# sczhou/Upscale-A-Video

Hardware: NVIDIA H100
Metric: upscaled frames/sec (30 DDIM steps, 180x320->4x) (higher is better)
Workload: dtype f16

## Files before the change

### upscale_a_video_b200/csrc/igemm.cu

```cuda
#include <stdarg.h>
#include <stdlib.h>
#include <stdio.h>
#include <string.h>

#include <atomic>
#include <mutex>

#include "uav_common.cuh"

namespace uav {

static thread_local char g_err[1024] = "";
void set_last_error(const char* fmt, ...) {
  va_list ap;
  va_start(ap, fmt);
  vsnprintf(g_err, sizeof(g_err), fmt, ap);
  va_end(ap);
}
std::atomic<uint64_t> g_launches{0};

int current_device() {
  int dev = 0;
  cudaGetDevice(&dev);
  return dev;
}

int num_sms() {
  static int n[64] = {0};
  const int dev = current_device() & 63;
  if (n[dev] == 0) {
    int v = 0;
    cudaDeviceGetAttribute(&v, cudaDevAttrMultiProcessorCount, dev);
    n[dev] = v > 0 ? v : 132;
  }
  return n[dev];
}

PFN_encodeTiled get_encode_tiled() {
  static PFN_encodeTiled fn = nullptr;
  static std::once_flag once;
  std::call_once(once, [] {
    void* p = nullptr;
    cudaDriverEntryPointQueryResult qres;
    if (cudaGetDriverEntryPoint("cuTensorMapEncodeTiled", &p, cudaEnableDefault, &qres) ==
            cudaSuccess &&
        qres == cudaDriverEntryPointSuccess)
      fn = reinterpret_cast<PFN_encodeTiled>(p);
  });
  return fn;
}

constexpr int BLOCK_M = 128;
constexpr int BLOCK_K = 64;
constexpr int MAX_TAPS = 49;
constexpr int NUM_THREADS = 384;
constexpr int NUM_EPI_THREADS = 256;
constexpr int A_STAGE_BYTES = BLOCK_M * BLOCK_K * 2;
constexpr int SLAB_BYTES = BLOCK_M * 128;
constexpr int SMEM_LIMIT = 232448;

struct alignas(64) IgemmParams {
  CUtensorMap map_a;
  CUtensorMap map_b;
  CUtensorMap map_out;
  CUtensorMap map_res;
  int32_t tap_off[MAX_TAPS][5];
  int32_t num_taps;
  int32_t kblocks_per_tap;
  int32_t k_per_tap;
  uint32_t box[5];
  uint32_t tiles[5];
  uint32_t out_dims[5];
  uint32_t n_tiles, num_tiles;
  int32_t N;
  int32_t n_out;
  int32_t tma_store;
  int32_t res_tma;
  const float* bias;
  const __half* rowvec;
  int64_t rows_per_vec, ld_rowvec;
  const __half* residual;
  int64_t ld_res;
  int32_t act, out_dtype;
  int64_t ld_out;
  void* out;
  float out_scale;
  float* gn_partial;
  int64_t gn_blocks;
};

template <int BLOCK_N, bool GEGLU>
struct IgemmCfg {
  static constexpr int OUT_TILE_N = GEGLU ? BLOCK_N / 2 : BLOCK_N;
  static constexpr int B_STAGE_BYTES = BLOCK_N * BLOCK_K * 2;
  static constexpr int STAGE_BYTES = A_STAGE_BYTES + B_STAGE_BYTES;
  static constexpr int STAGING_BYTES = (OUT_TILE_N >= 64) ? (OUT_TILE_N / 64) * SLAB_BYTES : 0;
  static constexpr int AUX_BYTES = 1024;
  static constexpr int STAGES_RAW = (SMEM_LIMIT - 1024 - STAGING_BYTES - AUX_BYTES) / STAGE_BYTES;
  static constexpr int STAGES = STAGES_RAW > 8 ? 8 : STAGES_RAW;
  static constexpr int SMEM_BYTES = STAGES * STAGE_BYTES + STAGING_BYTES + AUX_BYTES + 1024 ;
  static constexpr int ACC = BLOCK_N / 2;
};

__device__ __forceinline__ void epi_bar_sync() {
  asm volatile("bar.sync 1, %0;" ::"n"(NUM_EPI_THREADS) : "memory");
}
__device__ __forceinline__ float apply_act(float x, int act) {
  switch (act) {
    case UAV_ACT_SILU: return silu_f(x);
    case UAV_ACT_RELU: return fmaxf(x, 0.f);
    case UAV_ACT_SIGMOID: return rcp_ftz(1.0f + ex2_ftz(-1.4426950408889634f * x));
    case UAV_ACT_TANH: return 1.0f - 2.0f * rcp_ftz(1.0f + ex2_ftz(2.8853900817779268f * x));
    case UAV_ACT_GELU: return gelu_erf_f(x);
    case UAV_ACT_QUICK_GELU: return x * rcp_ftz(1.0f + ex2_ftz(-2.4554669595930156f * x));
    default: return x;
  }
}
__device__ __forceinline__ float warp_sum(float v) {
#pragma unroll
  for (int o = 16; o >= 1; o >>= 1) v += __shfl_xor_sync(0xffffffffu, v, o);
  return v;
}

template <int BLOCK_N, bool GEGLU, bool TMA_EPI, bool AUX>
__global__ void __launch_bounds__(NUM_THREADS, 1)
    igemm_kernel(const __grid_constant__ IgemmParams p) {
  using Cfg = IgemmCfg<BLOCK_N, GEGLU>;
  static_assert(!TMA_EPI || Cfg::OUT_TILE_N >= 64, "TMA-store epilogue needs >= 64-column output tiles");
  constexpr int OUT_TILE_N = Cfg::OUT_TILE_N;
  constexpr int STAGES = Cfg::STAGES;
  extern __shared__ uint8_t smem_raw[];
  const uint32_t raw_addr = smem_u32(smem_raw);
  uint8_t* smem = smem_raw + (((raw_addr + 1023u) & ~1023u) - raw_addr);
  uint8_t* staging = smem + STAGES * Cfg::STAGE_BYTES;
  uint64_t* bars = reinterpret_cast<uint64_t*>(staging + Cfg::STAGING_BYTES);
  uint64_t* full_bar = bars;
  uint64_t* empty_bar = bars + STAGES;
  uint64_t* res_bar = bars + 2 * STAGES;

  const int warp_idx = threadIdx.x >> 5;
  const int lane = threadIdx.x & 31;

  if (threadIdx.x == 0) {
    tma_prefetch_desc(&p.map_a);
    tma_prefetch_desc(&p.map_b);
    if (TMA_EPI) tma_prefetch_desc(&p.map_out);
    if (TMA_EPI && p.res_tma) tma_prefetch_desc(&p.map_res);
    for (int s = 0; s < STAGES; ++s) {
      mbar_init(&full_bar[s], 1);
      mbar_init(&empty_bar[s], NUM_EPI_THREADS / 32);
    }
    mbar_init(res_bar, 1);
    fence_barrier_init();
  }
  __syncthreads();
  const int num_kb = p.num_taps * p.kblocks_per_tap;

  if (warp_idx < 4) {
    if (threadIdx.x == 0) {
      int stage = 0;
      uint32_t phase = 0;
      for (uint32_t w = blockIdx.x; w < p.num_tiles; w += gridDim.x) {
        const uint32_t n_tile = w % p.n_tiles;
        uint32_t idx = w / p.n_tiles;
        const int c1 = (idx % p.tiles[1]) * p.box[1];
        idx /= p.tiles[1];
        const int c2 = (idx % p.tiles[2]) * p.box[2];
        idx /= p.tiles[2];
        const int c3 = (idx % p.tiles[3]) * p.box[3];
        idx /= p.tiles[3];
        const int c4 = idx * p.box[4];
        for (int tap = 0; tap < p.num_taps; ++tap) {
          const int o0 = p.tap_off[tap][0], o1 = p.tap_off[tap][1], o2 = p.tap_off[tap][2],
                    o3 = p.tap_off[tap][3], o4 = p.tap_off[tap][4];
          for (int kc = 0; kc < p.kblocks_per_tap; ++kc) {
            mbar_wait(&empty_bar[stage], phase ^ 1);
            uint8_t* sa = smem + stage * Cfg::STAGE_BYTES;
            uint8_t* sb = sa + A_STAGE_BYTES;
            mbar_expect_tx(&full_bar[stage], Cfg::STAGE_BYTES);
            tma_load_5d(&p.map_a, &full_bar[stage], sa, kc * BLOCK_K + o0, c1 + o1, c2 + o2, c3 + o3, c4 + o4);
            const int kcoord = tap * p.k_per_tap + kc * BLOCK_K;
            if (GEGLU) {
              tma_load_2d(&p.map_b, &full_bar[stage], sb, kcoord, n_tile * (BLOCK_N / 2));
              tma_load_2d(&p.map_b, &full_bar[stage], sb + Cfg::B_STAGE_BYTES / 2, kcoord,
                          p.N / 2 + n_tile * (BLOCK_N / 2));
            } else {
              tma_load_2d(&p.map_b, &full_bar[stage], sb, kcoord, n_tile * BLOCK_N);
            }
            if (++stage == STAGES) {
              stage = 0;
              phase ^= 1;
            }
          }
        }
      }
    }
    return;
  }

  const int et = threadIdx.x - 128;
  const int wg = et >> 7;
  const int cw = et >> 5;
  const int lq = lane >> 2, lr = lane & 3;
  uint32_t lrow[2], l1[2], l2[2], l3[2], l4[2];
#pragma unroll
  for (int h = 0; h < 2; ++h) {
    uint32_t r = 16 * cw + lq + 8 * h;
    lrow[h] = r;
    l1[h] = r % p.box[1];
    r /= p.box[1];
    l2[h] = r % p.box[2];
    r /= p.box[2];
    l3[h] = r % p.box[3];
    r /= p.box[3];
    l4[h] = r;
  }
  int stage = 0;
  uint32_t phase = 0, res_phase = 0;
  float acc[Cfg::ACC];
#pragma unroll
  for (int i = 0; i < Cfg::ACC; ++i) acc[i] = 0.f;

  for (uint32_t w = blockIdx.x; w < p.num_tiles; w += gridDim.x) {
    const uint32_t n_tile = w % p.n_tiles;
    const uint32_t m_tile = w / p.n_tiles;
    uint32_t idx = m_tile;
    const uint32_t t1 = (idx % p.tiles[1]) * p.box[1];
    idx /= p.tiles[1];
    const uint32_t t2 = (idx % p.tiles[2]) * p.box[2];
    idx /= p.tiles[2];
    const uint32_t t3 = (idx % p.tiles[3]) * p.box[3];
    idx /= p.tiles[3];
    const uint32_t t4 = idx * p.box[4];
    const int n_base = n_tile * OUT_TILE_N;

    if constexpr (TMA_EPI) {
      if (et == 0) {
        asm volatile("cp.async.bulk.wait_group.read 0;" ::: "memory");
        if (AUX && p.res_tma) {
          uint32_t bytes = 0;
#pragma unroll
          for (int sl = 0; sl < OUT_TILE_N / 64; ++sl)
            if (n_base + sl * 64 < p.n_out) bytes += SLAB_BYTES;
          mbar_expect_tx(res_bar, bytes);
#pragma unroll
          for (int sl = 0; sl < OUT_TILE_N / 64; ++sl)
            if (n_base + sl * 64 < p.n_out)
              tma_load_5d(&p.map_res, res_bar, staging + sl * SLAB_BYTES, n_base + sl * 64, (int)t1, (int)t2, (int)t3,
                          (int)t4);
        }
      }
    }

    int prev = 0;
    for (int kb = 0; kb < num_kb; ++kb) {
      mbar_wait(&full_bar[stage], phase);
      const uint32_t sa = smem_u32(smem + stage * Cfg::STAGE_BYTES) + wg * (64 * 128);
      const uint32_t sb = smem_u32(smem + stage * Cfg::STAGE_BYTES + A_STAGE_BYTES);
      const uint64_t adesc = gmma_desc_sw128(sa), bdesc = gmma_desc_sw128(sb);
      wgmma_fence();
#pragma unroll
      for (int k = 0; k < BLOCK_K / 16; ++k) wgmma_ss(acc, adesc + 2 * k, bdesc + 2 * k, (kb | k) != 0);
      wgmma_commit();
      if (kb > 0) {
        wgmma_wait<1>();
        if (lane == 0) mbar_arrive(&empty_bar[prev]);
      }
      prev = stage;
      if (++stage == STAGES) {
        stage = 0;
        phase ^= 1;
      }
    }
    wgmma_wait<0>();
    wgmma_fence_operands(acc);
    if (lane == 0) mbar_arrive(&empty_bar[prev]);

    bool row_ok[2];
    int64_t out_row[2];
    const __half* rv[2];
    const __half* res[2];
#pragma unroll
    for (int h = 0; h < 2; ++h) {
      const uint32_t o1 = t1 + l1[h], o2 = t2 + l2[h], o3 = t3 + l3[h], o4 = t4 + l4[h];
      row_ok[h] = o1 < p.out_dims[1] && o2 < p.out_dims[2] && o3 < p.out_dims[3] && o4 < p.out_dims[4];
      out_row[h] = ((static_cast<int64_t>(o4) * p.out_dims[3] + o3) * p.out_dims[2] + o2) * p.out_dims[1] + o1;
      rv[h] = (AUX && p.rowvec != nullptr && row_ok[h]) ? p.rowvec + (out_row[h] / p.rows_per_vec) * p.ld_rowvec
                                                         : nullptr;
      res[h] = (AUX && !TMA_EPI && p.residual != nullptr && row_ok[h]) ? p.residual + out_row[h] * p.ld_res : nullptr;
    }
    if constexpr (TMA_EPI) {
      epi_bar_sync();
      if constexpr (AUX) {
        if (p.res_tma) {
          mbar_wait(res_bar, res_phase);
          res_phase ^= 1;
        }
      }
    }
#pragma unroll
    for (int jb = 0; jb < OUT_TILE_N / 8; ++jb) {
      const int col = jb * 8 + 2 * lr;
      const int n = n_base + col;
      const bool ok0 = n < p.n_out, ok1 = n + 1 < p.n_out;
      float b0 = 0.f, b1 = 0.f, g0 = 0.f, g1 = 0.f;
      if (p.bias != nullptr) {
        if (ok0) b0 = __ldg(p.bias + n);
        if (ok1) b1 = __ldg(p.bias + n + 1);
        if (GEGLU) {
          if (ok0) g0 = __ldg(p.bias + p.N / 2 + n);
          if (ok1) g1 = __ldg(p.bias + p.N / 2 + n + 1);
        }
      }
      float gs = 0.f, gq = 0.f;
#pragma unroll
      for (int h = 0; h < 2; ++h) {
        const float a0 = acc[4 * jb + 2 * h], a1 = acc[4 * jb + 2 * h + 1];
        float x0, x1;
        if constexpr (GEGLU) {
          constexpr int GJ = OUT_TILE_N / 8;
          const float q0 = acc[4 * (jb + GJ) + 2 * h], q1 = acc[4 * (jb + GJ) + 2 * h + 1];
          x0 = (a0 + b0) * gelu_erf_f(q0 + g0);
          x1 = (a1 + b1) * gelu_erf_f(q1 + g1);
        } else {
          x0 = a0 + b0;
          x1 = a1 + b1;
        }
        const uint32_t row = lrow[h];
        uint8_t* sp = staging + (col >> 6) * SLAB_BYTES + row * 128 + ((((col & 63) >> 3) ^ (row & 7)) << 4) + (col & 7) * 2;
        if constexpr (AUX) {
          if (rv[h] != nullptr) {
            if (ok0) x0 += __half2float(rv[h][n]);
            if (ok1) x1 += __half2float(rv[h][n + 1]);
          }
          if (p.act != UAV_ACT_NONE) {
            x0 = apply_act(x0, p.act);
            x1 = apply_act(x1, p.act);
          }
          if (TMA_EPI && p.res_tma) {
            const float2 r = __half22float2(*reinterpret_cast<const __half2*>(sp));
            x0 = fmaf(x0, p.out_scale, r.x);
            x1 = fmaf(x1, p.out_scale, r.y);
          } else if (res[h] != nullptr) {
            x0 = fmaf(x0, p.out_scale, ok0 ? __half2float(res[h][n]) : 0.f);
            x1 = fmaf(x1, p.out_scale, ok1 ? __half2float(res[h][n + 1]) : 0.f);
          } else if (p.out_scale != 1.0f) {
            x0 *= p.out_scale;
            x1 *= p.out_scale;
          }
          if (row_ok[h] && ok0) {
            gs += x0 + x1;
            gq = fmaf(x0, x0, fmaf(x1, x1, gq));
          }
        }
        if constexpr (TMA_EPI) {
          *reinterpret_cast<uint32_t*>(sp) = pack_half2_sat(x0, x1);
        } else if (row_ok[h]) {
          if (p.out_dtype == UAV_F16) {
            __half* op = reinterpret_cast<__half*>(p.out) + out_row[h] * p.ld_out + n;
            if (ok0) op[0] = __float2half_rn(fminf(fmaxf(x0, -65504.f), 65504.f));
            if (ok1) op[1] = __float2half_rn(fminf(fmaxf(x1, -65504.f), 65504.f));
          } else {
            float* op = reinterpret_cast<float*>(p.out) + out_row[h] * p.ld_out + n;
            if (ok0) op[0] = x0;
            if (ok1) op[1] = x1;
          }
        }
      }
      if constexpr (AUX && TMA_EPI) {
        if (p.gn_partial != nullptr) {
          gs = warp_sum(gs);
          gq = warp_sum(gq);
          const int oct = (n_base >> 3) + jb;
          const int64_t blk = static_cast<int64_t>(m_tile) * 8 + cw;
          if (lane == 0 && blk < p.gn_blocks && oct * 8 < p.n_out) {
            p.gn_partial[(static_cast<int64_t>(oct) * p.gn_blocks + blk) * 2] = gs;
            p.gn_partial[(static_cast<int64_t>(oct) * p.gn_blocks + blk) * 2 + 1] = gq;
          }
        }
      }
    }
    if constexpr (TMA_EPI) {
      fence_proxy_async();
      epi_bar_sync();
      if (et == 0) {
#pragma unroll
        for (int sl = 0; sl < OUT_TILE_N / 64; ++sl) {
          if (n_base + sl * 64 < p.n_out) {
            asm volatile(
                "cp.async.bulk.tensor.5d.global.shared::cta.bulk_group"
                " [%0, {%2, %3, %4, %5, %6}], [%1];" ::"l"(reinterpret_cast<uint64_t>(&p.map_out)),
                "r"(smem_u32(staging + sl * SLAB_BYTES)), "r"(n_base + sl * 64), "r"(t1), "r"(t2), "r"(t3), "r"(t4)
                : "memory");
          }
        }
        asm volatile("cp.async.bulk.commit_group;" ::: "memory");
      }
    }
  }
  if (TMA_EPI && et == 0) asm volatile("cp.async.bulk.wait_group.read 0;" ::: "memory");
}

struct IgemmDesc {
  const void* a;
  int rank_a;
  uint64_t a_dims[5];
  uint64_t a_strides[5];
  uint32_t box[5];
  uint32_t tiles[5];
  uint32_t out_dims[5];
  int num_taps;
  int32_t tap_off[MAX_TAPS][5];
  int k_per_tap;
  const void* w;
  int64_t N;
  void* out;
  const uav_epilogue_t* epi;
  uint64_t out_strides[5];
};

template <int BLOCK_N, bool GEGLU, bool TMA_EPI, bool AUX>
static uav_status_t launch_instance2(IgemmParams& p, cudaStream_t stream) {
  using Cfg = IgemmCfg<BLOCK_N, GEGLU>;
  static uint64_t configured = 0;
  const uint64_t dev_bit = 1ull << (current_device() & 63);
  auto kern = igemm_kernel<BLOCK_N, GEGLU, TMA_EPI, AUX>;
  if (!(configured & dev_bit)) {
    UAV_CHECK_CUDA(cudaFuncSetAttribute(kern, cudaFuncAttributeMaxDynamicSharedMemorySize, Cfg::SMEM_BYTES));
    configured |= dev_bit;
  }
  const uint32_t sms = (uint32_t)num_sms();
  kern<<<p.num_tiles < sms ? p.num_tiles : sms, NUM_THREADS, Cfg::SMEM_BYTES, stream>>>(p);
  UAV_CHECK_CUDA(cudaGetLastError());
  g_launches.fetch_add(1, std::memory_order_relaxed);
  return UAV_OK;
}

template <int BLOCK_N, bool GEGLU>
static uav_status_t launch_instance(IgemmParams& p, cudaStream_t stream) {
  const bool aux = p.rowvec != nullptr || p.residual != nullptr || (p.act != UAV_ACT_NONE && p.act != UAV_ACT_GEGLU) ||
                   p.out_scale != 1.0f || p.gn_partial != nullptr;
  if constexpr (IgemmCfg<BLOCK_N, GEGLU>::OUT_TILE_N >= 64) {
    if (p.tma_store) {
      return aux ? launch_instance2<BLOCK_N, GEGLU, true, true>(p, stream)
                 : launch_instance2<BLOCK_N, GEGLU, true, false>(p, stream);
    }
  }
  return launch_instance2<BLOCK_N, GEGLU, false, true>(p, stream);
}

static uav_status_t launch_igemm(const IgemmDesc& d, cudaStream_t stream) {
  const uav_epilogue_t* e = d.epi;
  UAV_REQUIRE(e != nullptr, "igemm: epilogue descriptor is NULL");
  UAV_REQUIRE(d.a && d.w && d.out, "igemm: null pointer");
  UAV_REQUIRE(d.k_per_tap > 0 && d.k_per_tap % 8 == 0,
              "igemm: input channels (%d) must be a positive multiple of 8", d.k_per_tap);
  UAV_REQUIRE((reinterpret_cast<uintptr_t>(d.a) & 15) == 0 &&
                  (reinterpret_cast<uintptr_t>(d.w) & 15) == 0,
              "igemm: operands must be 16-byte aligned");
  const bool geglu = e->act == UAV_ACT_GEGLU;
  UAV_REQUIRE(!geglu || (d.N % 128 == 0), "igemm: GEGLU needs N %% 128 == 0 (N=%lld)",
              (long long)d.N);
  PFN_encodeTiled encode = get_encode_tiled();
  UAV_REQUIRE(encode != nullptr, "igemm: cuTensorMapEncodeTiled entry point unavailable");

  IgemmParams p;
  memset(&p, 0, sizeof(p));
  int block_n;
  if (geglu || d.N > 64) block_n = 128;
  else if (d.N > 32) block_n = 64;
  else if (d.N > 16) block_n = 32;
  else block_n = 16;

  {
    cuuint64_t dims[5], strides[4];
    cuuint32_t box[5], estr[5] = {1, 1, 1, 1, 1};
    for (int i = 0; i < 5; ++i) {
      dims[i] = d.a_dims[i];
      box[i] = d.box[i];
      UAV_REQUIRE(dims[i] >= 1 && box[i] >= 1 && box[i] <= 256, "igemm: bad A dim/box %d", i);
    }
    for (int i = 1; i < 5; ++i) {
      strides[i - 1] = d.a_strides[i] * 2;
      UAV_REQUIRE(strides[i - 1] % 16 == 0, "igemm: A stride %d not 16-byte aligned", i);
    }
    CUresult r = encode(&p.map_a, CU_TENSOR_MAP_DATA_TYPE_FLOAT16, 5, const_cast<void*>(d.a),
                        dims, strides, box, estr, CU_TENSOR_MAP_INTERLEAVE_NONE,
                        CU_TENSOR_MAP_SWIZZLE_128B, CU_TENSOR_MAP_L2_PROMOTION_L2_256B,
                        CU_TENSOR_MAP_FLOAT_OOB_FILL_NONE);
    UAV_REQUIRE(r == CUDA_SUCCESS, "igemm: cuTensorMapEncodeTiled(A) failed with %d", (int)r);
  }
  const int64_t k_total = (int64_t)d.num_taps * d.k_per_tap;
  {
    cuuint64_t dims[2] = {(cuuint64_t)k_total, (cuuint64_t)d.N};
    cuuint64_t strides[1] = {(cuuint64_t)k_total * 2};
    cuuint32_t box[2] = {64, (cuuint32_t)(geglu ? block_n / 2 : block_n)};
    cuuint32_t estr[2] = {1, 1};
    CUresult r = encode(&p.map_b, CU_TENSOR_MAP_DATA_TYPE_FLOAT16, 2, const_cast<void*>(d.w), dims,
                        strides, box, estr, CU_TENSOR_MAP_INTERLEAVE_NONE,
                        CU_TENSOR_MAP_SWIZZLE_128B, CU_TENSOR_MAP_L2_PROMOTION_L2_256B,
                        CU_TENSOR_MAP_FLOAT_OOB_FILL_NONE);
    UAV_REQUIRE(r == CUDA_SUCCESS, "igemm: cuTensorMapEncodeTiled(B) failed with %d", (int)r);
  }
  UAV_REQUIRE(d.num_taps >= 1 && d.num_taps <= MAX_TAPS, "igemm: bad tap count %d", d.num_taps);
  memcpy(p.tap_off, d.tap_off, sizeof(int32_t) * 5 * d.num_taps);
  p.num_taps = d.num_taps;
  p.k_per_tap = d.k_per_tap;
  p.kblocks_per_tap = (d.k_per_tap + BLOCK_K - 1) / BLOCK_K;
  uint64_t m_tiles = 1;
  uint32_t box_prod = 1;
  for (int i = 0; i < 5; ++i) {
    p.box[i] = d.box[i];
    p.tiles[i] = d.tiles[i];
    p.out_dims[i] = d.out_dims[i];
    if (i >= 1) {
      m_tiles *= d.tiles[i];
      box_prod *= d.box[i];
    }
  }
  UAV_REQUIRE(box_prod == BLOCK_M && d.box[0] == 64, "igemm: M-tile box must cover 128 rows");
  p.N = (int32_t)d.N;
  p.n_out = (int32_t)(geglu ? d.N / 2 : d.N);
  const int out_tile_n = geglu ? block_n / 2 : block_n;
  p.n_tiles = (uint32_t)((p.n_out + out_tile_n - 1) / out_tile_n);
  UAV_REQUIRE(m_tiles * p.n_tiles < (1ull << 31), "igemm: too many tiles");
  p.num_tiles = (uint32_t)(m_tiles * p.n_tiles);
  auto aligned16 = [](const void* q) { return (reinterpret_cast<uintptr_t>(q) & 15) == 0; };
  const bool can_tma = out_tile_n >= 64 && e->out_dtype == UAV_F16 && p.n_out % 8 == 0 && e->ld_out % 8 == 0 &&
                       aligned16(d.out) &&
                       (e->residual == nullptr || (e->ld_res % 8 == 0 && aligned16(e->residual))) &&
                       (e->rowvec == nullptr || (e->ld_rowvec % 8 == 0 && aligned16(e->rowvec)));
  p.res_tma = (can_tma && e->residual != nullptr) ? 1 : 0;
  p.bias = e->bias;
  p.rowvec = reinterpret_cast<const __half*>(e->rowvec);
  p.rows_per_vec = e->rows_per_vec > 0 ? e->rows_per_vec : 1;
  p.ld_rowvec = e->ld_rowvec;
  p.residual = reinterpret_cast<const __half*>(e->residual);
  p.ld_res = e->ld_res;
  p.act = e->act;
  p.out_dtype = e->out_dtype;
  p.ld_out = e->ld_out;
  p.out = d.out;
  p.out_scale = e->out_scale == 0.0f ? 1.0f : e->out_scale;
  p.gn_partial = reinterpret_cast<float*>(e->gn_partial);
  p.gn_blocks = e->gn_blocks;
  UAV_REQUIRE(!(geglu && p.out_scale != 1.0f), "igemm: out_scale is not supported with GEGLU");
  UAV_REQUIRE(p.ld_out >= p.n_out, "igemm: ld_out (%lld) < output columns (%d)",
              (long long)p.ld_out, p.n_out);
  UAV_REQUIRE(e->out_dtype == UAV_F16 || e->out_dtype == UAV_F32, "igemm: bad out_dtype");
  UAV_REQUIRE(e->act >= UAV_ACT_NONE && e->act <= UAV_ACT_QUICK_GELU, "igemm: bad activation");
  if (p.num_tiles == 0) return UAV_OK;

  p.tma_store = can_tma ? 1 : 0;
  if (p.gn_partial != nullptr) {
    UAV_REQUIRE(can_tma && !geglu && d.out_strides[1] == 0,
                "igemm: GroupNorm statistics need the dense fp16 TMA-store epilogue (n_out >= 33, 16-byte aligned) without GEGLU");
    UAV_REQUIRE(p.gn_blocks == (int64_t)m_tiles * 8, "igemm: gn_blocks is %lld, this launch produces %lld blocks",
                (long long)p.gn_blocks, (long long)m_tiles * 8);
  }
  UAV_REQUIRE(d.out_strides[1] == 0 || (can_tma && p.residual == nullptr && p.rowvec == nullptr),
              "igemm: a strided output view needs the TMA-store epilogue without residual / row vector");
  if (can_tma) {
    cuuint64_t dims[5], strides[4];
    cuuint32_t box[5], estr[5] = {1, 1, 1, 1, 1};
    dims[0] = (cuuint64_t)p.n_out;
    box[0] = 64;
    uint64_t stride_el = (uint64_t)p.ld_out;
    for (int i = 1; i < 5; ++i) {
      dims[i] = d.out_dims[i];
      box[i] = d.box[i];
      strides[i - 1] = (d.out_strides[i] ? d.out_strides[i] : stride_el) * 2;
      stride_el *= d.out_dims[i];
    }
    CUresult r = encode(&p.map_out, CU_TENSOR_MAP_DATA_TYPE_FLOAT16, 5, d.out, dims, strides, box,
                        estr, CU_TENSOR_MAP_INTERLEAVE_NONE, CU_TENSOR_MAP_SWIZZLE_128B,
                        CU_TENSOR_MAP_L2_PROMOTION_NONE, CU_TENSOR_MAP_FLOAT_OOB_FILL_NONE);
    UAV_REQUIRE(r == CUDA_SUCCESS, "igemm: cuTensorMapEncodeTiled(out) failed with %d", (int)r);
    if (p.res_tma) {
      uint64_t rs = (uint64_t)p.ld_res;
      for (int i = 1; i < 5; ++i) {
        strides[i - 1] = rs * 2;
        rs *= d.out_dims[i];
      }
      r = encode(&p.map_res, CU_TENSOR_MAP_DATA_TYPE_FLOAT16, 5, const_cast<__half*>(p.residual), dims, strides, box, estr,
                 CU_TENSOR_MAP_INTERLEAVE_NONE, CU_TENSOR_MAP_SWIZZLE_128B, CU_TENSOR_MAP_L2_PROMOTION_L2_256B,
                 CU_TENSOR_MAP_FLOAT_OOB_FILL_NONE);
      UAV_REQUIRE(r == CUDA_SUCCESS, "igemm: cuTensorMapEncodeTiled(residual) failed with %d", (int)r);
    }
  }

  if (geglu) return launch_instance<128, true>(p, stream);
  switch (block_n) {
    case 128: return launch_instance<128, false>(p, stream);
    case 64: return launch_instance<64, false>(p, stream);
    case 32: return launch_instance<32, false>(p, stream);
    default: return launch_instance<16, false>(p, stream);
  }
}

static void pick_tile_2d(int64_t W, int64_t H, uint32_t* tw, uint32_t* th) {
  int64_t best = -1;
  for (uint32_t w = 128; w >= 1; w >>= 1) {
    const uint32_t h = 128 / w;
    const int64_t cover = ((W + w - 1) / w) * w * ((H + h - 1) / h) * h;
    if (best < 0 || cover < best) {
      best = cover;
      *tw = w;
      *th = h;
    }
  }
}

}

using namespace uav;

extern "C" {

int64_t uav_gn_partial_blocks(int64_t w, int64_t h, int64_t images) {
  if (w <= 0 || h <= 0 || images <= 0) return 0;
  if (h == 1) return ((w + 127) / 128) * images * 8;
  uint32_t tw, th;
  pick_tile_2d(w, h, &tw, &th);
  return ((w + tw - 1) / tw) * ((h + th - 1) / th) * images * 8;
}

const char* uav_version(void) { return "uav_b200 0.3 (sm_90a)"; }
const char* uav_last_error_string(void) { return g_err; }
uint64_t uav_launch_count(void) { return g_launches.load(); }

uav_status_t uav_linear(const void* a, int64_t M, int64_t K, int64_t lda, const void* w,
                        int64_t N, void* out, const uav_epilogue_t* epi, uav_stream_t stream) {
  UAV_REQUIRE(M >= 0 && K > 0 && N > 0 && lda >= K, "uav_linear: bad shape");
  if (M == 0) return UAV_OK;
  IgemmDesc d;
  memset(&d, 0, sizeof(d));
  d.a = a;
  const uint64_t dims[5] = {(uint64_t)K, (uint64_t)M, 1, 1, 1};
  const uint64_t strides[5] = {1, (uint64_t)lda, (uint64_t)lda * M, (uint64_t)lda * M,
                               (uint64_t)lda * M};
  const uint32_t box[5] = {64, 128, 1, 1, 1};
  for (int i = 0; i < 5; ++i) {
    d.a_dims[i] = dims[i];
    d.a_strides[i] = strides[i];
    d.box[i] = box[i];
    d.tiles[i] = 1;
    d.out_dims[i] = 1;
  }
  d.tiles[1] = (uint32_t)((M + 127) / 128);
  d.out_dims[1] = (uint32_t)M;
  d.num_taps = 1;
  d.k_per_tap = (int)K;
  d.w = w;
  d.N = N;
  d.out = out;
  d.epi = epi;
  return launch_igemm(d, (cudaStream_t)stream);
}

uav_status_t uav_conv2d(const void* x, int64_t NB, int64_t H, int64_t W, int64_t Cin,
                        int64_t ld_in, const void* w, int64_t Cout, int ksize, int stride,
                        int pad_mode, void* out, const uav_epilogue_t* epi,
                        uav_stream_t stream) {
  UAV_REQUIRE(NB > 0 && H > 0 && W > 0 && Cin > 0 && Cout > 0 && ld_in >= Cin,
              "uav_conv2d: bad shape");
  UAV_REQUIRE(ksize == 1 || ksize == 3, "uav_conv2d: ksize must be 1 or 3");
  UAV_REQUIRE(stride == 1 || stride == 2, "uav_conv2d: stride must be 1 or 2");
  UAV_REQUIRE(pad_mode == 0 || (pad_mode == 1 && stride == 2 && ksize == 3),
              "uav_conv2d: pad_mode 1 needs a stride-2 3x3 conv");
  if (ksize == 1 && stride == 1) return uav_linear(x, NB * H * W, Cin, ld_in, w, Cout, out, epi, stream);
  IgemmDesc d;
  memset(&d, 0, sizeof(d));
  d.a = x;
  d.w = w;
  d.N = Cout;
  d.out = out;
  d.epi = epi;
  d.k_per_tap = (int)Cin;
  const int pad = ksize / 2;
  if (stride == 1) {
    uint32_t tw, th;
    pick_tile_2d(W, H, &tw, &th);
    const uint64_t dims[5] = {(uint64_t)Cin, (uint64_t)W, (uint64_t)H, (uint64_t)NB, 1};
    const uint64_t strides[5] = {1, (uint64_t)ld_in, (uint64_t)ld_in * W,
                                 (uint64_t)ld_in * W * H, (uint64_t)ld_in * W * H * NB};
    const uint32_t box[5] = {64, tw, th, 1, 1};
    const uint32_t tiles[5] = {1, (uint32_t)((W + tw - 1) / tw), (uint32_t)((H + th - 1) / th),
                               (uint32_t)NB, 1};
    const uint32_t odims[5] = {1, (uint32_t)W, (uint32_t)H, (uint32_t)NB, 1};
    for (int i = 0; i < 5; ++i) {
      d.a_dims[i] = dims[i];
      d.a_strides[i] = strides[i];
      d.box[i] = box[i];
      d.tiles[i] = tiles[i];
      d.out_dims[i] = odims[i];
    }
    d.num_taps = ksize * ksize;
    for (int ky = 0; ky < ksize; ++ky)
      for (int kx = 0; kx < ksize; ++kx) {
        int32_t* o = d.tap_off[ky * ksize + kx];
        o[0] = 0;
        o[1] = kx - pad;
        o[2] = ky - pad;
        o[3] = 0;
        o[4] = 0;
      }
  } else {
    UAV_REQUIRE(H % 2 == 0 && W % 2 == 0, "uav_conv2d: stride 2 needs even H, W (got %lldx%lld)",
                (long long)H, (long long)W);
    UAV_REQUIRE(ld_in == Cin, "uav_conv2d: stride 2 needs a dense input (ld_in == Cin)");
    const int64_t Wo = W / 2, Ho = H / 2;
    uint32_t tw, th;
    pick_tile_2d(Wo, Ho, &tw, &th);
    const uint64_t dims[5] = {(uint64_t)(2 * Cin), (uint64_t)Wo, 2, (uint64_t)Ho, (uint64_t)NB};
    const uint64_t strides[5] = {1, (uint64_t)(2 * Cin), (uint64_t)(W * Cin),
                                 (uint64_t)(2 * W * Cin), (uint64_t)(H * W * Cin)};
    const uint32_t box[5] = {64, tw, 1, th, 1};
    const uint32_t tiles[5] = {1, (uint32_t)((Wo + tw - 1) / tw), 1,
                               (uint32_t)((Ho + th - 1) / th), (uint32_t)NB};
    const uint32_t odims[5] = {1, (uint32_t)Wo, 1, (uint32_t)Ho, (uint32_t)NB};
    for (int i = 0; i < 5; ++i) {
      d.a_dims[i] = dims[i];
      d.a_strides[i] = strides[i];
      d.box[i] = box[i];
      d.tiles[i] = tiles[i];
      d.out_dims[i] = odims[i];
    }
    d.num_taps = 9;
    for (int ky = 0; ky < 3; ++ky)
      for (int kx = 0; kx < 3; ++kx) {
        const int iy = ky - (pad_mode == 0 ? 1 : 0);
        const int ix = kx - (pad_mode == 0 ? 1 : 0);
        const int py = ((iy % 2) + 2) % 2, px = ((ix % 2) + 2) % 2;
        const int oy = (iy - py) / 2, ox = (ix - px) / 2;
        int32_t* o = d.tap_off[ky * 3 + kx];
        o[0] = px * (int)Cin;
        o[1] = ox;
        o[2] = py;
        o[3] = oy;
        o[4] = 0;
      }
  }
  return launch_igemm(d, (cudaStream_t)stream);
}

// ... 180 lines not shown
```

### upscale_a_video_b200/csrc/uav_common.cuh

```cuda
#pragma once
#include <cuda_runtime.h>
#include <cuda_fp16.h>
#include <cuda.h>
#include <stdint.h>

#include "../../include/uav_b200.h"

namespace uav {

void set_last_error(const char* fmt, ...);
#define UAV_CHECK_CUDA(expr)                                                             \
  do {                                                                                   \
    cudaError_t _e = (expr);                                                             \
    if (_e != cudaSuccess) {                                                             \
      uav::set_last_error("%s:%d: %s -> %s", __FILE__, __LINE__, #expr,                  \
                          cudaGetErrorString(_e));                                       \
      return UAV_ERR_CUDA;                                                               \
    }                                                                                    \
  } while (0)
#define UAV_REQUIRE(cond, ...)                                                           \
  do {                                                                                   \
    if (!(cond)) {                                                                       \
      uav::set_last_error(__VA_ARGS__);                                                  \
      return UAV_ERR_INVALID;                                                            \
    }                                                                                    \
  } while (0)

int num_sms();
int current_device();

__device__ __forceinline__ uint32_t smem_u32(const void* p) {
  return static_cast<uint32_t>(__cvta_generic_to_shared(p));
}

__device__ __forceinline__ void mbar_init(uint64_t* bar, uint32_t count) {
  asm volatile("mbarrier.init.shared::cta.b64 [%0], %1;" ::"r"(smem_u32(bar)), "r"(count));
}
__device__ __forceinline__ void fence_barrier_init() {
  asm volatile("fence.mbarrier_init.release.cluster;" ::: "memory");
}
__device__ __forceinline__ void fence_proxy_async() {
  asm volatile("fence.proxy.async.shared::cta;" ::: "memory");
}
__device__ __forceinline__ void mbar_expect_tx(uint64_t* bar, uint32_t bytes) {
  asm volatile("mbarrier.arrive.expect_tx.shared::cta.b64 _, [%0], %1;" ::"r"(smem_u32(bar)),
               "r"(bytes)
               : "memory");
}
__device__ __forceinline__ void mbar_arrive(uint64_t* bar) {
  asm volatile("mbarrier.arrive.shared::cta.b64 _, [%0];" ::"r"(smem_u32(bar)) : "memory");
}
__device__ __forceinline__ void mbar_wait(uint64_t* bar, uint32_t parity) {
  asm volatile(
      "{\n\t"
      ".reg .pred P1;\n\t"
      "LAB_WAIT:\n\t"
      "mbarrier.try_wait.parity.shared::cta.b64 P1, [%0], %1, %2;\n\t"
      "@P1 bra DONE;\n\t"
      "bra LAB_WAIT;\n\t"
      "DONE:\n\t"
      "}\n" ::"r"(smem_u32(bar)),
      "r"(parity), "r"(0x989680u)
      : "memory");
}

__device__ __forceinline__ void tma_prefetch_desc(const void* desc) {
  asm volatile("prefetch.tensormap [%0];" ::"l"(reinterpret_cast<uint64_t>(desc)) : "memory");
}
__device__ __forceinline__ void tma_load_2d(const void* desc, uint64_t* bar, void* smem, int c0,
                                            int c1) {
  asm volatile(
      "cp.async.bulk.tensor.2d.shared::cluster.global.mbarrier::complete_tx::bytes"
      " [%0], [%1, {%3, %4}], [%2];" ::"r"(smem_u32(smem)),
      "l"(reinterpret_cast<uint64_t>(desc)), "r"(smem_u32(bar)), "r"(c0), "r"(c1)
      : "memory");
}
__device__ __forceinline__ void tma_load_3d(const void* desc, uint64_t* bar, void* smem, int c0,
                                            int c1, int c2) {
  asm volatile(
      "cp.async.bulk.tensor.3d.shared::cluster.global.mbarrier::complete_tx::bytes"
      " [%0], [%1, {%3, %4, %5}], [%2];" ::"r"(smem_u32(smem)),
      "l"(reinterpret_cast<uint64_t>(desc)), "r"(smem_u32(bar)), "r"(c0), "r"(c1), "r"(c2)
      : "memory");
}
__device__ __forceinline__ void tma_load_5d(const void* desc, uint64_t* bar, void* smem, int c0,
                                            int c1, int c2, int c3, int c4) {
  asm volatile(
      "cp.async.bulk.tensor.5d.shared::cluster.global.mbarrier::complete_tx::bytes"
      " [%0], [%1, {%3, %4, %5, %6, %7}], [%2];" ::"r"(smem_u32(smem)),
      "l"(reinterpret_cast<uint64_t>(desc)), "r"(smem_u32(bar)), "r"(c0), "r"(c1), "r"(c2),
      "r"(c3), "r"(c4)
      : "memory");
}


__device__ __forceinline__ void wgmma_fence() { asm volatile("wgmma.fence.sync.aligned;" ::: "memory"); }
__device__ __forceinline__ void wgmma_commit() { asm volatile("wgmma.commit_group.sync.aligned;" ::: "memory"); }
template <int N>
__device__ __forceinline__ void wgmma_wait() {
  asm volatile("wgmma.wait_group.sync.aligned %0;" ::"n"(N) : "memory");
}
template <int R>
__device__ __forceinline__ void wgmma_fence_operands(float (&d)[R]) {
#pragma unroll
  for (int i = 0; i < R; ++i) asm volatile("" : "+f"(d[i])::"memory");
}

__device__ __forceinline__ uint64_t gmma_desc_sw128(uint32_t smem_addr) {
  uint64_t d = 0;
  d |= static_cast<uint64_t>((smem_addr & 0x3FFFF) >> 4);
  d |= static_cast<uint64_t>(1) << 16;
  d |= static_cast<uint64_t>(1024 >> 4) << 32;
  d |= static_cast<uint64_t>(1) << 62;
  return d;
}


__device__ __forceinline__ void wgmma_ss(float (&d)[8], uint64_t adesc, uint64_t bdesc, uint32_t scale_d) {
  asm volatile(
      "{\n.reg .pred p;\n"
      "setp.ne.b32 p, %10, 0;\n"
      "wgmma.mma_async.sync.aligned.m64n16k16.f32.f16.f16 {%0, %1, %2, %3, %4, %5, %6, %7}, %8, %9, p, 1, 1, 0, 0;\n"
      "}\n"
      : "+f"(d[0]), "+f"(d[1]), "+f"(d[2]), "+f"(d[3]), "+f"(d[4]), "+f"(d[5]), "+f"(d[6]), "+f"(d[7])
      : "l"(adesc), "l"(bdesc), "r"(scale_d));
}
__device__ __forceinline__ void wgmma_ss(float (&d)[16], uint64_t adesc, uint64_t bdesc, uint32_t scale_d) {
  asm volatile(
      "{\n.reg .pred p;\n"
      "setp.ne.b32 p, %18, 0;\n"
      "wgmma.mma_async.sync.aligned.m64n32k16.f32.f16.f16 {%0, %1, %2, %3, %4, %5, %6, %7, %8, %9, %10, %11, %12, %13, %14, %15}, %16, %17, p, 1, 1, 0, 0;\n"
      "}\n"
      : "+f"(d[0]), "+f"(d[1]), "+f"(d[2]), "+f"(d[3]), "+f"(d[4]), "+f"(d[5]), "+f"(d[6]), "+f"(d[7]), "+f"(d[8]), "+f"(d[9]), "+f"(d[10]), "+f"(d[11]), "+f"(d[12]), "+f"(d[13]), "+f"(d[14]), "+f"(d[15])
      : "l"(adesc), "l"(bdesc), "r"(scale_d));
}
__device__ __forceinline__ void wgmma_ss(float (&d)[32], uint64_t adesc, uint64_t bdesc, uint32_t scale_d) {
  asm volatile(
      "{\n.reg .pred p;\n"
      "setp.ne.b32 p, %34, 0;\n"
      "wgmma.mma_async.sync.aligned.m64n64k16.f32.f16.f16 {%0, %1, %2, %3, %4, %5, %6, %7, %8, %9, %10, %11, %12, %13, %14, %15, %16, %17, %18, %19, %20, %21, %22, %23, %24, %25, %26, %27, %28, %29, %30, %31}, %32, %33, p, 1, 1, 0, 0;\n"
      "}\n"
      : "+f"(d[0]), "+f"(d[1]), "+f"(d[2]), "+f"(d[3]), "+f"(d[4]), "+f"(d[5]), "+f"(d[6]), "+f"(d[7]), "+f"(d[8]), "+f"(d[9]), "+f"(d[10]), "+f"(d[11]), "+f"(d[12]), "+f"(d[13]), "+f"(d[14]), "+f"(d[15]), "+f"(d[16]), "+f"(d[17]), "+f"(d[18]), "+f"(d[19]), "+f"(d[20]), "+f"(d[21]), "+f"(d[22]), "+f"(d[23]), "+f"(d[24]), "+f"(d[25]), "+f"(d[26]), "+f"(d[27]), "+f"(d[28]), "+f"(d[29]), "+f"(d[30]), "+f"(d[31])
      : "l"(adesc), "l"(bdesc), "r"(scale_d));
}
__device__ __forceinline__ void wgmma_ss(float (&d)[64], uint64_t adesc, uint64_t bdesc, uint32_t scale_d) {
  asm volatile(
      "{\n.reg .pred p;\n"
      "setp.ne.b32 p, %66, 0;\n"
      "wgmma.mma_async.sync.aligned.m64n128k16.f32.f16.f16 {%0, %1, %2, %3, %4, %5, %6, %7, %8, %9, %10, %11, %12, %13, %14, %15, %16, %17, %18, %19, %20, %21, %22, %23, %24, %25, %26, %27, %28, %29, %30, %31, %32, %33, %34, %35, %36, %37, %38, %39, %40, %41, %42, %43, %44, %45, %46, %47, %48, %49, %50, %51, %52, %53, %54, %55, %56, %57, %58, %59, %60, %61, %62, %63}, %64, %65, p, 1, 1, 0, 0;\n"
      "}\n"
      : "+f"(d[0]), "+f"(d[1]), "+f"(d[2]), "+f"(d[3]), "+f"(d[4]), "+f"(d[5]), "+f"(d[6]), "+f"(d[7]), "+f"(d[8]), "+f"(d[9]), "+f"(d[10]), "+f"(d[11]), "+f"(d[12]), "+f"(d[13]), "+f"(d[14]), "+f"(d[15]), "+f"(d[16]), "+f"(d[17]), "+f"(d[18]), "+f"(d[19]), "+f"(d[20]), "+f"(d[21]), "+f"(d[22]), "+f"(d[23]), "+f"(d[24]), "+f"(d[25]), "+f"(d[26]), "+f"(d[27]), "+f"(d[28]), "+f"(d[29]), "+f"(d[30]), "+f"(d[31]), "+f"(d[32]), "+f"(d[33]), "+f"(d[34]), "+f"(d[35]), "+f"(d[36]), "+f"(d[37]), "+f"(d[38]), "+f"(d[39]), "+f"(d[40]), "+f"(d[41]), "+f"(d[42]), "+f"(d[43]), "+f"(d[44]), "+f"(d[45]), "+f"(d[46]), "+f"(d[47]), "+f"(d[48]), "+f"(d[49]), "+f"(d[50]), "+f"(d[51]), "+f"(d[52]), "+f"(d[53]), "+f"(d[54]), "+f"(d[55]), "+f"(d[56]), "+f"(d[57]), "+f"(d[58]), "+f"(d[59]), "+f"(d[60]), "+f"(d[61]), "+f"(d[62]), "+f"(d[63])
      : "l"(adesc), "l"(bdesc), "r"(scale_d));
}
__device__ __forceinline__ void wgmma_rs_tb(float (&d)[32], const uint32_t (&a)[4], uint64_t bdesc, uint32_t scale_d) {
  asm volatile(
      "{\n.reg .pred p;\n"
      "setp.ne.b32 p, %37, 0;\n"
      "wgmma.mma_async.sync.aligned.m64n64k16.f32.f16.f16 {%0, %1, %2, %3, %4, %5, %6, %7, %8, %9, %10, %11, %12, %13, %14, %15, %16, %17, %18, %19, %20, %21, %22, %23, %24, %25, %26, %27, %28, %29, %30, %31}, {%32, %33, %34, %35}, %36, p, 1, 1, 1;\n"
      "}\n"
      : "+f"(d[0]), "+f"(d[1]), "+f"(d[2]), "+f"(d[3]), "+f"(d[4]), "+f"(d[5]), "+f"(d[6]), "+f"(d[7]), "+f"(d[8]), "+f"(d[9]), "+f"(d[10]), "+f"(d[11]), "+f"(d[12]), "+f"(d[13]), "+f"(d[14]), "+f"(d[15]), "+f"(d[16]), "+f"(d[17]), "+f"(d[18]), "+f"(d[19]), "+f"(d[20]), "+f"(d[21]), "+f"(d[22]), "+f"(d[23]), "+f"(d[24]), "+f"(d[25]), "+f"(d[26]), "+f"(d[27]), "+f"(d[28]), "+f"(d[29]), "+f"(d[30]), "+f"(d[31])
      : "r"(a[0]), "r"(a[1]), "r"(a[2]), "r"(a[3]), "l"(bdesc), "r"(scale_d));
}

__device__ __forceinline__ float ex2_ftz(float x) {
  float r;
  asm("ex2.approx.ftz.f32 %0, %1;" : "=f"(r) : "f"(x));
  return r;
}
__device__ __forceinline__ float rcp_ftz(float x) {
  float r;
  asm("rcp.approx.ftz.f32 %0, %1;" : "=f"(r) : "f"(x));
  return r;
}
__device__ __forceinline__ float silu_f(float x) { return x * rcp_ftz(1.0f + ex2_ftz(-1.4426950408889634f * x)); }
__device__ __forceinline__ void silu2_f(float& a, float& b) {
  const float d0 = 1.0f + ex2_ftz(fminf(-1.4426950408889634f * a, 60.0f));
  const float d1 = 1.0f + ex2_ftz(fminf(-1.4426950408889634f * b, 60.0f));
  const float r = rcp_ftz(d0 * d1);
  a *= r * d1;
  b *= r * d0;
}
__device__ __forceinline__ float gelu_erf_f(float x) {
  const float ax = fminf(fabsf(x), 6.0f);
  const float t = fmaf(ax, 0.3333333333333333f, -1.0f);
  float p = -0.005517261102795601f;
  p = fmaf(p, t, -0.012404678389430046f);
  p = fmaf(p, t, 0.020884426310658455f);
  p = fmaf(p, t, -0.02991572767496109f);
  p = fmaf(p, t, 0.09405267238616943f);
  p = fmaf(p, t, -0.2069002389907837f);
  p = fmaf(p, t, -6.035426616668701f);
  p = fmaf(p, t, -14.20971965789795f);
  p = fmaf(p, t, -9.532933235168457f);
  return fmaf(-ax, ex2_ftz(p), fmaxf(x, 0.0f));
}

__device__ __forceinline__ uint32_t pack_half2_sat(float a, float b) {
  uint32_t r;
  asm("cvt.rn.satfinite.f16x2.f32 %0, %1, %2;" : "=r"(r) : "f"(b), "f"(a));
  return r;
}

__device__ __forceinline__ uint4 ldg16(const void* p) {
  return *reinterpret_cast<const uint4*>(p);
}
__device__ __forceinline__ void stg16(void* p, const uint4& v) {
  *reinterpret_cast<uint4*>(p) = v;
}

typedef CUresult (*PFN_encodeTiled)(CUtensorMap*, CUtensorMapDataType, cuuint32_t, void*,
                                    const cuuint64_t*, const cuuint64_t*, const cuuint32_t*,
                                    const cuuint32_t*, CUtensorMapInterleave, CUtensorMapSwizzle,
                                    CUtensorMapL2promotion, CUtensorMapFloatOOBfill);
PFN_encodeTiled get_encode_tiled();

}
```

Measured before the change: 0.7759.

## Add 256-wide N tiles to implicit GEMM with register rebalancing

Adds a BLOCK_N=256 instantiation that uses the m64n256k16 wgmma for GEGLU and multi-tap convolutions with wide N. A wave-count heuristic picks the wide tile only when it pays off. To fit the larger accumulators, producer warps give up registers via setmaxnreg and consumer warps take more. The epilogue is split into passes of up to 128 columns with accumulator shifting. The aim is more A-tile reuse per load and fewer tiles, at the cost of register pressure, fewer pipeline stages and possible spills.

```diff
diff --git a/upscale_a_video_b200/csrc/igemm.cu b/upscale_a_video_b200/csrc/igemm.cu
--- a/upscale_a_video_b200/csrc/igemm.cu
+++ b/upscale_a_video_b200/csrc/igemm.cu
@@ -100,6 +100,7 @@
   static constexpr int STAGES = STAGES_RAW > 8 ? 8 : STAGES_RAW;
   static constexpr int SMEM_BYTES = STAGES * STAGE_BYTES + STAGING_BYTES + AUX_BYTES + 1024 ;
   static constexpr int ACC = BLOCK_N / 2;
+  static_assert(SMEM_BYTES <= SMEM_LIMIT, "stage ring + output staging exceed the shared memory of a block");
 };
 
 __device__ __forceinline__ void epi_bar_sync() {
@@ -157,6 +158,7 @@
   const int num_kb = p.num_taps * p.kblocks_per_tap;
 
   if (warp_idx < 4) {
+    asm volatile("setmaxnreg.dec.sync.aligned.u32 40;" ::: "memory");
     if (threadIdx.x == 0) {
       int stage = 0;
       uint32_t phase = 0;
@@ -198,6 +200,7 @@
     return;
   }
 
+  asm volatile("setmaxnreg.inc.sync.aligned.u32 232;" ::: "memory");
   const int et = threadIdx.x - 128;
   const int wg = et >> 7;
   const int cw = et >> 5;
@@ -298,86 +301,95 @@
         }
       }
     }
-#pragma unroll
-    for (int jb = 0; jb < OUT_TILE_N / 8; ++jb) {
-      const int col = jb * 8 + 2 * lr;
-      const int n = n_base + col;
-      const bool ok0 = n < p.n_out, ok1 = n + 1 < p.n_out;
-      float b0 = 0.f, b1 = 0.f, g0 = 0.f, g1 = 0.f;
-      if (p.bias != nullptr) {
-        if (ok0) b0 = __ldg(p.bias + n);
-        if (ok1) b1 = __ldg(p.bias + n + 1);
-        if (GEGLU) {
-          if (ok0) g0 = __ldg(p.bias + p.N / 2 + n);
-          if (ok1) g1 = __ldg(p.bias + p.N / 2 + n + 1);
-        }
-      }
-      float gs = 0.f, gq = 0.f;
-#pragma unroll
-      for (int h = 0; h < 2; ++h) {
-        const float a0 = acc[4 * jb + 2 * h], a1 = acc[4 * jb + 2 * h + 1];
-        float x0, x1;
-        if constexpr (GEGLU) {
-          constexpr int GJ = OUT_TILE_N / 8;
-          const float q0 = acc[4 * (jb + GJ) + 2 * h], q1 = acc[4 * (jb + GJ) + 2 * h + 1];
-          x0 = (a0 + b0) * gelu_erf_f(q0 + g0);
-          x1 = (a1 + b1) * gelu_erf_f(q1 + g1);
-        } else {
-          x0 = a0 + b0;
-          x1 = a1 + b1;
-        }
-        const uint32_t row = lrow[h];
-        uint8_t* sp = staging + (col >> 6) * SLAB_BYTES + row * 128 + ((((col & 63) >> 3) ^ (row & 7)) << 4) + (col & 7) * 2;
-        if constexpr (AUX) {
-          if (rv[h] != nullptr) {
-            if (ok0) x0 += __half2float(rv[h][n]);
-            if (ok1) x1 += __half2float(rv[h][n + 1]);
-          }
-          if (p.act != UAV_ACT_NONE) {
-            x0 = apply_act(x0, p.act);
-            x1 = apply_act(x1, p.act);
-          }
-          if (TMA_EPI && p.res_tma) {
-            const float2 r = __half22float2(*reinterpret_cast<const __half2*>(sp));
-            x0 = fmaf(x0, p.out_scale, r.x);
-            x1 = fmaf(x1, p.out_scale, r.y);
-          } else if (res[h] != nullptr) {
-            x0 = fmaf(x0, p.out_scale, ok0 ? __half2float(res[h][n]) : 0.f);
-            x1 = fmaf(x1, p.out_scale, ok1 ? __half2float(res[h][n + 1]) : 0.f);
-          } else if (p.out_scale != 1.0f) {
-            x0 *= p.out_scale;
-            x1 *= p.out_scale;
-          }
-          if (row_ok[h] && ok0) {
-            gs += x0 + x1;
-            gq = fmaf(x0, x0, fmaf(x1, x1, gq));
+    constexpr int EPI_N = GEGLU ? OUT_TILE_N : (OUT_TILE_N < 128 ? OUT_TILE_N : 128);
+    constexpr int EPI_ACC = EPI_N / 2;
+#pragma unroll 1
+    for (int pass = 0; pass < OUT_TILE_N / EPI_N; ++pass) {
+#pragma unroll
+      for (int jb = 0; jb < EPI_N / 8; ++jb) {
+        const int col = pass * EPI_N + jb * 8 + 2 * lr;
+        const int n = n_base + col;
+        const bool ok0 = n < p.n_out, ok1 = n + 1 < p.n_out;
+        float b0 = 0.f, b1 = 0.f, g0 = 0.f, g1 = 0.f;
+        if (p.bias != nullptr) {
+          if (ok0) b0 = __ldg(p.bias + n);
+          if (ok1) b1 = __ldg(p.bias + n + 1);
+          if (GEGLU) {
+            if (ok0) g0 = __ldg(p.bias + p.N / 2 + n);
+            if (ok1) g1 = __ldg(p.bias + p.N / 2 + n + 1);
           }
         }
-        if constexpr (TMA_EPI) {
-          *reinterpret_cast<uint32_t*>(sp) = pack_half2_sat(x0, x1);
-        } else if (row_ok[h]) {
-          if (p.out_dtype == UAV_F16) {
-            __half* op = reinterpret_cast<__half*>(p.out) + out_row[h] * p.ld_out + n;
-            if (ok0) op[0] = __float2half_rn(fminf(fmaxf(x0, -65504.f), 65504.f));
-            if (ok1) op[1] = __float2half_rn(fminf(fmaxf(x1, -65504.f), 65504.f));
+        float gs = 0.f, gq = 0.f;
+#pragma unroll
+        for (int h = 0; h < 2; ++h) {
+          const float a0 = acc[4 * jb + 2 * h], a1 = acc[4 * jb + 2 * h + 1];
+          float x0, x1;
+          if constexpr (GEGLU) {
+            constexpr int GJ = OUT_TILE_N / 8;
+            const float q0 = acc[4 * (jb + GJ) + 2 * h], q1 = acc[4 * (jb + GJ) + 2 * h + 1];
+            x0 = (a0 + b0) * gelu_erf_f(q0 + g0);
+            x1 = (a1 + b1) * gelu_erf_f(q1 + g1);
           } else {
-            float* op = reinterpret_cast<float*>(p.out) + out_row[h] * p.ld_out + n;
-            if (ok0) op[0] = x0;
-            if (ok1) op[1] = x1;
+            x0 = a0 + b0;
+            x1 = a1 + b1;
+          }
+          const uint32_t row = lrow[h];
+          uint8_t* sp = staging + (col >> 6) * SLAB_BYTES + row * 128 + ((((col & 63) >> 3) ^ (row & 7)) << 4) + (col & 7) * 2;
+          if constexpr (AUX) {
+            if (rv[h] != nullptr) {
+              if (ok0) x0 += __half2float(rv[h][n]);
+              if (ok1) x1 += __half2float(rv[h][n + 1]);
+            }
+            if (p.act != UAV_ACT_NONE) {
+              x0 = apply_act(x0, p.act);
+              x1 = apply_act(x1, p.act);
+            }
+            if (TMA_EPI && p.res_tma) {
+              const float2 r = __half22float2(*reinterpret_cast<const __half2*>(sp));
+              x0 = fmaf(x0, p.out_scale, r.x);
+              x1 = fmaf(x1, p.out_scale, r.y);
+            } else if (res[h] != nullptr) {
+              x0 = fmaf(x0, p.out_scale, ok0 ? __half2float(res[h][n]) : 0.f);
+              x1 = fmaf(x1, p.out_scale, ok1 ? __half2float(res[h][n + 1]) : 0.f);
+            } else if (p.out_scale != 1.0f) {
+              x0 *= p.out_scale;
+              x1 *= p.out_scale;
+            }
+            if (row_ok[h] && ok0) {
+              gs += x0 + x1;
+              gq = fmaf(x0, x0, fmaf(x1, x1, gq));
+            }
+          }
+          if constexpr (TMA_EPI) {
+            *reinterpret_cast<uint32_t*>(sp) = pack_half2_sat(x0, x1);
+          } else if (row_ok[h]) {
+            if (p.out_dtype == UAV_F16) {
+              __half* op = reinterpret_cast<__half*>(p.out) + out_row[h] * p.ld_out + n;
+              if (ok0) op[0] = __float2half_rn(fminf(fmaxf(x0, -65504.f), 65504.f));
+              if (ok1) op[1] = __float2half_rn(fminf(fmaxf(x1, -65504.f), 65504.f));
+            } else {
+              float* op = reinterpret_cast<float*>(p.out) + out_row[h] * p.ld_out + n;
+              if (ok0) op[0] = x0;
+              if (ok1) op[1] = x1;
+            }
           }
         }
-      }
-      if constexpr (AUX && TMA_EPI) {
-        if (p.gn_partial != nullptr) {
-          gs = warp_sum(gs);
-          gq = warp_sum(gq);
-          const int oct = (n_base >> 3) + jb;
-          const int64_t blk = static_cast<int64_t>(m_tile) * 8 + cw;
-          if (lane == 0 && blk < p.gn_blocks && oct * 8 < p.n_out) {
-            p.gn_partial[(static_cast<int64_t>(oct) * p.gn_blocks + blk) * 2] = gs;
-            p.gn_partial[(static_cast<int64_t>(oct) * p.gn_blocks + blk) * 2 + 1] = gq;
+        if constexpr (AUX && TMA_EPI) {
+          if (p.gn_partial != nullptr) {
+            gs = warp_sum(gs);
+            gq = warp_sum(gq);
+            const int oct = n >> 3;
+            const int64_t blk = static_cast<int64_t>(m_tile) * 8 + cw;
+            if (lane == 0 && blk < p.gn_blocks && oct * 8 < p.n_out) {
+              p.gn_partial[(static_cast<int64_t>(oct) * p.gn_blocks + blk) * 2] = gs;
+              p.gn_partial[(static_cast<int64_t>(oct) * p.gn_blocks + blk) * 2 + 1] = gq;
+            }
           }
         }
+      }
+      if (pass + 1 < OUT_TILE_N / EPI_N) {
+#pragma unroll
+        for (int i = 0; i + EPI_ACC < Cfg::ACC; ++i) acc[i] = acc[i + EPI_ACC];
       }
     }
     if constexpr (TMA_EPI) {
@@ -449,6 +461,15 @@
   return launch_instance2<BLOCK_N, GEGLU, false, true>(p, stream);
 }
 
+constexpr double WIDE_TILE_COST = 1.9;
+
+static bool wide_tile_pays(uint64_t m_tiles, int64_t n_out, int64_t out_wide) {
+  const uint64_t sms = (uint64_t)num_sms();
+  const uint64_t waves_wide = (m_tiles * ((n_out + out_wide - 1) / out_wide) + sms - 1) / sms;
+  const uint64_t waves_narrow = (m_tiles * ((2 * n_out + out_wide - 1) / out_wide) + sms - 1) / sms;
+  return (double)waves_wide * WIDE_TILE_COST < (double)waves_narrow;
+}
+
 static uav_status_t launch_igemm(const IgemmDesc& d, cudaStream_t stream) {
   const uav_epilogue_t* e = d.epi;
   UAV_REQUIRE(e != nullptr, "igemm: epilogue descriptor is NULL");
@@ -466,8 +487,13 @@
 
   IgemmParams p;
   memset(&p, 0, sizeof(p));
+  uint64_t m_tiles = 1;
+  for (int i = 1; i < 5; ++i) m_tiles *= d.tiles[i];
+  const int64_t n_out = geglu ? d.N / 2 : d.N;
   int block_n;
-  if (geglu || d.N > 64) block_n = 128;
+  if (geglu) block_n = (d.N % 256 == 0 && wide_tile_pays(m_tiles, n_out, 128)) ? 256 : 128;
+  else if (d.N >= 256 && d.num_taps > 1 && wide_tile_pays(m_tiles, n_out, 256)) block_n = 256;
+  else if (d.N > 64) block_n = 128;
   else if (d.N > 32) block_n = 64;
   else if (d.N > 16) block_n = 32;
   else block_n = 16;
@@ -507,20 +533,16 @@
   p.num_taps = d.num_taps;
   p.k_per_tap = d.k_per_tap;
   p.kblocks_per_tap = (d.k_per_tap + BLOCK_K - 1) / BLOCK_K;
-  uint64_t m_tiles = 1;
   uint32_t box_prod = 1;
   for (int i = 0; i < 5; ++i) {
     p.box[i] = d.box[i];
     p.tiles[i] = d.tiles[i];
     p.out_dims[i] = d.out_dims[i];
-    if (i >= 1) {
-      m_tiles *= d.tiles[i];
-      box_prod *= d.box[i];
-    }
+    if (i >= 1) box_prod *= d.box[i];
   }
   UAV_REQUIRE(box_prod == BLOCK_M && d.box[0] == 64, "igemm: M-tile box must cover 128 rows");
   p.N = (int32_t)d.N;
-  p.n_out = (int32_t)(geglu ? d.N / 2 : d.N);
+  p.n_out = (int32_t)n_out;
   const int out_tile_n = geglu ? block_n / 2 : block_n;
   p.n_tiles = (uint32_t)((p.n_out + out_tile_n - 1) / out_tile_n);
   UAV_REQUIRE(m_tiles * p.n_tiles < (1ull << 31), "igemm: too many tiles");
@@ -589,8 +611,9 @@
     }
   }
 
-  if (geglu) return launch_instance<128, true>(p, stream);
+  if (geglu) return block_n == 256 ? launch_instance<256, true>(p, stream) : launch_instance<128, true>(p, stream);
   switch (block_n) {
+    case 256: return launch_instance<256, false>(p, stream);
     case 128: return launch_instance<128, false>(p, stream);
     case 64: return launch_instance<64, false>(p, stream);
     case 32: return launch_instance<32, false>(p, stream);
diff --git a/upscale_a_video_b200/csrc/uav_common.cuh b/upscale_a_video_b200/csrc/uav_common.cuh
--- a/upscale_a_video_b200/csrc/uav_common.cuh
+++ b/upscale_a_video_b200/csrc/uav_common.cuh
@@ -152,6 +152,15 @@
       : "+f"(d[0]), "+f"(d[1]), "+f"(d[2]), "+f"(d[3]), "+f"(d[4]), "+f"(d[5]), "+f"(d[6]), "+f"(d[7]), "+f"(d[8]), "+f"(d[9]), "+f"(d[10]), "+f"(d[11]), "+f"(d[12]), "+f"(d[13]), "+f"(d[14]), "+f"(d[15]), "+f"(d[16]), "+f"(d[17]), "+f"(d[18]), "+f"(d[19]), "+f"(d[20]), "+f"(d[21]), "+f"(d[22]), "+f"(d[23]), "+f"(d[24]), "+f"(d[25]), "+f"(d[26]), "+f"(d[27]), "+f"(d[28]), "+f"(d[29]), "+f"(d[30]), "+f"(d[31]), "+f"(d[32]), "+f"(d[33]), "+f"(d[34]), "+f"(d[35]), "+f"(d[36]), "+f"(d[37]), "+f"(d[38]), "+f"(d[39]), "+f"(d[40]), "+f"(d[41]), "+f"(d[42]), "+f"(d[43]), "+f"(d[44]), "+f"(d[45]), "+f"(d[46]), "+f"(d[47]), "+f"(d[48]), "+f"(d[49]), "+f"(d[50]), "+f"(d[51]), "+f"(d[52]), "+f"(d[53]), "+f"(d[54]), "+f"(d[55]), "+f"(d[56]), "+f"(d[57]), "+f"(d[58]), "+f"(d[59]), "+f"(d[60]), "+f"(d[61]), "+f"(d[62]), "+f"(d[63])
       : "l"(adesc), "l"(bdesc), "r"(scale_d));
 }
+__device__ __forceinline__ void wgmma_ss(float (&d)[128], uint64_t adesc, uint64_t bdesc, uint32_t scale_d) {
+  asm volatile(
+      "{\n.reg .pred p;\n"
+      "setp.ne.b32 p, %130, 0;\n"
+      "wgmma.mma_async.sync.aligned.m64n256k16.f32.f16.f16 {%0, %1, %2, %3, %4, %5, %6, %7, %8, %9, %10, %11, %12, %13, %14, %15, %16, %17, %18, %19, %20, %21, %22, %23, %24, %25, %26, %27, %28, %29, %30, %31, %32, %33, %34, %35, %36, %37, %38, %39, %40, %41, %42, %43, %44, %45, %46, %47, %48, %49, %50, %51, %52, %53, %54, %55, %56, %57, %58, %59, %60, %61, %62, %63, %64, %65, %66, %67, %68, %69, %70, %71, %72, %73, %74, %75, %76, %77, %78, %79, %80, %81, %82, %83, %84, %85, %86, %87, %88, %89, %90, %91, %92, %93, %94, %95, %96, %97, %98, %99, %100, %101, %102, %103, %104, %105, %106, %107, %108, %109, %110, %111, %112, %113, %114, %115, %116, %117, %118, %119, %120, %121, %122, %123, %124, %125, %126, %127}, %128, %129, p, 1, 1, 0, 0;\n"
+      "}\n"
+      : "+f"(d[0]), "+f"(d[1]), "+f"(d[2]), "+f"(d[3]), "+f"(d[4]), "+f"(d[5]), "+f"(d[6]), "+f"(d[7]), "+f"(d[8]), "+f"(d[9]), "+f"(d[10]), "+f"(d[11]), "+f"(d[12]), "+f"(d[13]), "+f"(d[14]), "+f"(d[15]), "+f"(d[16]), "+f"(d[17]), "+f"(d[18]), "+f"(d[19]), "+f"(d[20]), "+f"(d[21]), "+f"(d[22]), "+f"(d[23]), "+f"(d[24]), "+f"(d[25]), "+f"(d[26]), "+f"(d[27]), "+f"(d[28]), "+f"(d[29]), "+f"(d[30]), "+f"(d[31]), "+f"(d[32]), "+f"(d[33]), "+f"(d[34]), "+f"(d[35]), "+f"(d[36]), "+f"(d[37]), "+f"(d[38]), "+f"(d[39]), "+f"(d[40]), "+f"(d[41]), "+f"(d[42]), "+f"(d[43]), "+f"(d[44]), "+f"(d[45]), "+f"(d[46]), "+f"(d[47]), "+f"(d[48]), "+f"(d[49]), "+f"(d[50]), "+f"(d[51]), "+f"(d[52]), "+f"(d[53]), "+f"(d[54]), "+f"(d[55]), "+f"(d[56]), "+f"(d[57]), "+f"(d[58]), "+f"(d[59]), "+f"(d[60]), "+f"(d[61]), "+f"(d[62]), "+f"(d[63]), "+f"(d[64]), "+f"(d[65]), "+f"(d[66]), "+f"(d[67]), "+f"(d[68]), "+f"(d[69]), "+f"(d[70]), "+f"(d[71]), "+f"(d[72]), "+f"(d[73]), "+f"(d[74]), "+f"(d[75]), "+f"(d[76]), "+f"(d[77]), "+f"(d[78]), "+f"(d[79]), "+f"(d[80]), "+f"(d[81]), "+f"(d[82]), "+f"(d[83]), "+f"(d[84]), "+f"(d[85]), "+f"(d[86]), "+f"(d[87]), "+f"(d[88]), "+f"(d[89]), "+f"(d[90]), "+f"(d[91]), "+f"(d[92]), "+f"(d[93]), "+f"(d[94]), "+f"(d[95]), "+f"(d[96]), "+f"(d[97]), "+f"(d[98]), "+f"(d[99]), "+f"(d[100]), "+f"(d[101]), "+f"(d[102]), "+f"(d[103]), "+f"(d[104]), "+f"(d[105]), "+f"(d[106]), "+f"(d[107]), "+f"(d[108]), "+f"(d[109]), "+f"(d[110]), "+f"(d[111]), "+f"(d[112]), "+f"(d[113]), "+f"(d[114]), "+f"(d[115]), "+f"(d[116]), "+f"(d[117]), "+f"(d[118]), "+f"(d[119]), "+f"(d[120]), "+f"(d[121]), "+f"(d[122]), "+f"(d[123]), "+f"(d[124]), "+f"(d[125]), "+f"(d[126]), "+f"(d[127])
+      : "l"(adesc), "l"(bdesc), "r"(scale_d));
+}
 __device__ __forceinline__ void wgmma_rs_tb(float (&d)[32], const uint32_t (&a)[4], uint64_t bdesc, uint32_t scale_d) {
   asm volatile(
       "{\n.reg .pred p;\n"
```

After: 0.8295 (median of 6 runs). 1.07x the previous value.
